# apcamargo/genomad

Hardware: NVIDIA H100
Metric: nn_classification_windows_per_s (higher is better)
Workload: dtype split operands on wgmma (conv: fp16 main pass + two e4m3 correction passes; w_v: 3 fp16 passes), fp32 accumulate; fp32-equivalent (<=1e-4 vs the fp32 oracle, measured ~1e-5)

## Files before the change

### genomad_b200/csrc/api.cu

```cuda
#include <cuda.h>
#include <cuda_runtime.h>
#include <cuda_fp16.h>

#include <algorithm>
#include <cmath>
#include <cstdio>
#include <cstring>
#include <string>
#include <vector>

#include "../../include/gnm.h"
#include "common.cuh"
#include "encode.cuh"
#include "conv_t.cuh"
#include "layer1_wv.cuh"
#include "conv_ref.cuh"
#include "igloo.cuh"
#include "dense.cuh"
#include "logits_tc.cuh"
#include "wv_gather.cuh"
#include "contigs.cuh"

using namespace gnm;

// ... 389 lines not shown
    if (dev_upload(h, &h->d1w, w->dense1_kernel, static_cast<size_t>(kHidden) * kHidden)) return 1;
    if (dev_upload(h, &h->d1b, w->dense1_bias, kHidden)) return 1;
    if (bn(w->bn1, &h->bn1_scale, &h->bn1_shift)) return 1;
    const float* dw[2] = {w->dense0_kernel, w->dense1_kernel};
    const int dk[2] = {256, kHidden};
    for (int L = 0; L < 2; ++L) {
      std::vector<float> thi(static_cast<size_t>(kHidden) * dk[L]), tlo(thi.size());
      for (int k = 0; k < dk[L]; ++k)
        for (int n = 0; n < kHidden; ++n)
          split_tf32(dw[L][static_cast<size_t>(k) * kHidden + n], thi[static_cast<size_t>(n) * dk[L] + k], tlo[static_cast<size_t>(n) * dk[L] + k]);
      if (dev_upload(h, &h->dwT_hi[L], thi.data(), thi.size())) return 1;
      if (dev_upload(h, &h->dwT_lo[L], tlo.data(), tlo.size())) return 1;
    }
    if (dev_upload(h, &h->d2w, w->dense2_kernel, static_cast<size_t>(kHidden) * 3)) return 1;
    if (dev_upload(h, &h->d2b, w->dense2_bias, 3)) return 1;
  }
  const size_t mb = static_cast<size_t>(max_batch);
  h->mb_pad = (max_batch + kBandWins - 1) / kBandWins * kBandWins;
  const size_t mbp = static_cast<size_t>(h->mb_pad);
  for (int i = 0; i < 2; ++i) {
    if (dev_alloc(h, &h->ybuf[i], mbp * kTok * kRowBytes)) return 1;
    for (int par = 0; par < 2; ++par) {
      if (dev_alloc(h, &h->q_set[par][i], mb * kPooled * kC)) return 1;
      if (dev_alloc(h, &h->mpi_set[par][i], mb * kPatches)) return 1;
      if (dev_alloc(h, &h->mpi_hi_set[par][i], mb * kPatches)) return 1;
      if (dev_alloc(h, &h->mpi_lo_set[par][i], mb * kPatches)) return 1;
    }
    h->q[i] = h->q_set[0][i]; h->mpi[i] = h->mpi_set[0][i]; h->mpi_hi[i] = h->mpi_hi_set[0][i]; h->mpi_lo[i] = h->mpi_lo_set[0][i];
    if (dev_alloc(h, &h->in_stage[i], mb * kWindow)) return 1;
    if (dev_alloc(h, &h->out_stage[i], mb * 3)) return 1;
    GNM_CUDA(cudaEventCreateWithFlags(&h->in_ready[i], cudaEventDisableTiming));
    GNM_CUDA(cudaEventCreateWithFlags(&h->in_free[i], cudaEventDisableTiming));
  }
  if (dev_alloc(h, &h->conv_dbg, static_cast<size_t>(h->num_sms) * 8)) return 1;
  GNM_CUDA(cudaMemset(h->conv_dbg, 0, static_cast<size_t>(h->num_sms) * 8 * sizeof(long long)));
  if (dev_alloc(h, &h->part, mbp * kGsSlots)) return 1;
  if (dev_alloc(h, &h->cta_split, static_cast<size_t>(2) * (h->num_sms + 1))) return 1;
  if (dev_alloc(h, &h->logits, mb * kLogitsLd)) return 1;
  if (dev_alloc(h, &h->logits_part, mb * kLogitsLd * kLgSplits)) return 1;
  if (dev_alloc(h, &h->h0, mb * 256)) return 1;
  if (dev_alloc(h, &h->h1, mb * kHidden)) return 1;
  if (dev_alloc(h, &h->h2, mb * kHidden)) return 1;
  if (dev_alloc(h, &h->hA_hi[0], mb * 256)) return 1;
  if (dev_alloc(h, &h->hA_lo[0], mb * 256)) return 1;
  if (dev_alloc(h, &h->hA_hi[1], mb * kHidden)) return 1;
  if (dev_alloc(h, &h->hA_lo[1], mb * kHidden)) return 1;
  GNM_CUDA(cudaStreamCreateWithFlags(&h->copy_stream, cudaStreamNonBlocking));
  GNM_CUDA(cudaStreamCreateWithFlags(&h->compute_stream, cudaStreamNonBlocking));
  {
    int prio_lo = 0, prio_hi = 0;
    GNM_CUDA(cudaDeviceGetStreamPriorityRange(&prio_lo, &prio_hi));
    GNM_CUDA(cudaStreamCreateWithPriority(&h->tail_stream, cudaStreamNonBlocking, prio_hi));
    for (int i = 0; i < 2; ++i) {
      GNM_CUDA(cudaEventCreateWithFlags(&h->main_done[i], cudaEventDisableTiming));
      GNM_CUDA(cudaEventCreateWithFlags(&h->tail_done[i], cudaEventDisableTiming));
    }
  }
  GNM_CUDA(cudaHostAlloc(reinterpret_cast<void**>(&h->status), sizeof(DeviceStatus), cudaHostAllocMapped));
  std::memset(h->status, 0, sizeof(DeviceStatus));

  PFN_encodeTiled enc = nullptr;
  if (get_encode_fn(&enc)) return 1;
  for (int i = 0; i < 2; ++i) {
    if (make_act_map(enc, &h->tm_act[i], h->ybuf[i], max_batch)) return 1;
    if (make_band_map(enc, &h->tm_band[i], h->ybuf[i], h->mb_pad)) return 1;
  }
  for (int i = 0; i < 4; ++i) {
    const int n_stages = i < 2 ? kConvStages : kWvStages;
// ... 90 lines not shown
    cfg.blockDim = dim3(kConvThreads); cfg.dynamicSmemBytes = kConvTSmem; cfg.stream = st; cfg.attrs = attr; cfg.numAttrs = 1;
    cfg.gridDim = dim3(grid / h->conv_cluster * h->conv_cluster);
    int max_clusters = 0;
    if (cudaOccupancyMaxActiveClusters(&max_clusters, conv_t_kernel<false>, &cfg) == cudaSuccess && max_clusters > 0)
      grid = std::min(grid / h->conv_cluster, max_clusters) * h->conv_cluster;
    else
      grid = grid / h->conv_cluster * h->conv_cluster;
    cfg.gridDim = dim3(grid);
    GNM_CUDA(cudaLaunchKernelEx(&cfg, conv_t_kernel<false>, h->tm_act[in_buf], h->tm_w_half[layer], p));
    return check_launch(h, "conv_t_kernel<false>(cluster)");
  }
  conv_t_kernel<false><<<grid, kConvThreads, kConvTSmem, st>>>(h->tm_act[in_buf], h->tm_w_half[layer], p);
  return check_launch(h, "conv_t_kernel<false>");
}
static int launch_wv_tc(gnm_handle* h, int s, int buf, int n, cudaStream_t st) {
  ConvTcParams p;
  p.status = h->status;
  p.experiment = 0;
  p.dbg = nullptr;
  p.bias = nullptr; p.y_out = nullptr; p.q_out = h->q[s];
  p.out_scale = h->wv_out_scale[s];
  p.out_fp8 = 0;
  p.n_tiles = n * kUnitsPerWin;
  const int grid = std::min(h->num_sms, p.n_tiles);
  conv_t_kernel<true><<<grid, kConvThreads, kConvTSmem, st>>>(h->tm_act[buf], h->tm_w_half[2 + s], p);
  return check_launch(h, "conv_t_kernel<true>");
}

static int wv_split(gnm_handle* h, int s, int groups, int grid, cudaStream_t st) {
  if (h->split_groups[s] == groups && h->split_grid[s] == grid) return 0;
  std::vector<double> cost(kNumBands);
  double total = 0;
  for (int b = 0; b < kNumBands; ++b) {
    const int per_warp = (h->band_groups[s][b] + kWgWarps - 1) / kWgWarps;
    cost[b] = h->wv_cost_base + h->wv_cost_group * per_warp;
    total += cost[b] * groups;
  }
  std::vector<int32_t>& sp = h->split_host[s];
  sp.assign(h->num_sms + 1, kNumBands * groups);
  sp[0] = 0;
  double acc = 0;
  int c = 1;
  for (int b = 0; b < kNumBands && c < grid; ++b)
    for (int g = 0; g < groups && c < grid; ++g) {
      acc += cost[b];
      if (acc >= total * c / grid) sp[c++] = b * groups + g + 1;
    }
  for (; c <= grid; ++c) sp[c] = kNumBands * groups;
  for (int i = 1; i <= grid; ++i) sp[i] = std::max(sp[i], sp[i - 1]);
  GNM_CUDA(cudaMemcpyAsync(h->cta_split + s * (h->num_sms + 1), sp.data(), (grid + 1) * sizeof(int32_t), cudaMemcpyHostToDevice, st));
  h->split_groups[s] = groups; h->split_grid[s] = grid;
  return 0;
}

static int launch_wv_gather(gnm_handle* h, int s, int buf, int n, cudaStream_t st) {
  WvGatherParams p;
  p.q_out = h->q[s]; p.out_scale = h->wv_out_scale[s];
  p.grp = h->grp[s]; p.band_gstart = h->band_gstart[s]; p.wfrag = h->wfrag[s]; p.gather_unscale = h->gather_unscale[s]; p.part_t = h->part;
  p.n_windows = n;
  p.n_pad = (n + kBandWins - 1) / kBandWins * kBandWins;
  p.groups = p.n_pad / kBandWins;
  p.n_units = kNumBands * p.groups;
  p.status = h->status;
  p.experiment = h->conv_experiment;
  p.dbg = (h->conv_experiment & 512) && s == 1 ? h->conv_dbg : nullptr;
  const int grid = std::min(h->num_sms, p.n_units);
  if (wv_split(h, s, p.groups, grid, st)) return 1;
// ... 535 lines not shown
  if (ns < 2) return 0;
  GNM_CUDA(cudaEventSynchronize(h->timer.events[ns - 1]));
  int k = 0;
  for (int i = 0; i + 1 < ns && k < cap; ++i) {
    if (std::strcmp(h->timer.names[i], "end") == 0) continue;
    float t = 0.f;
    GNM_CUDA(cudaEventElapsedTime(&t, h->timer.events[i], h->timer.events[i + 1]));
    if (names) names[k] = h->timer.names[i];
    if (ms) ms[k] = t;
    ++k;
  }
  *count = k;
  return 0;
}

extern "C" int gnm_debug_fetch(gnm_handle* h, const char* which, int n, float* d_dst, void* stream) {
  if (!h || !which || !d_dst) return fail("null argument");
  if (n < 1 || n > h->max_batch) return fail("gnm_debug_fetch: n out of range");
  GNM_CUDA(cudaSetDevice(h->device));
  cudaStream_t st = static_cast<cudaStream_t>(stream);
  const std::string k(which);
  const float* src = nullptr;
  size_t count = 0;
  if (k == "buf0" || k == "buf1") {
    const size_t rows = static_cast<size_t>(n) * kTok;
    join_rows_kernel<<<static_cast<unsigned>((rows * kC + 255) / 256), 256, 0, st>>>(h->ybuf[k == "buf1"], d_dst, rows,
                                                                                     h->ybuf_fp8lo[k == "buf1"]);
    return check_launch(h, "join_rows_kernel");
  } else if (k == "q0" || k == "q1") { src = h->q[k == "q1"]; count = static_cast<size_t>(n) * kPooled * kC; }
  else if (k == "mpi0" || k == "mpi1") { src = h->mpi[k == "mpi1"]; count = static_cast<size_t>(n) * kPatches; }
  else if (k == "h0") { src = h->h0; count = static_cast<size_t>(n) * 256; }
  else if (k == "h1" || k == "h2") { src = k == "h1" ? h->h1 : h->h2; count = static_cast<size_t>(n) * kHidden; }
  else if (k == "logits") { src = h->logits; count = static_cast<size_t>(n) * kLogitsLd; }
  else if (k == "conv_dbg") { src = reinterpret_cast<const float*>(h->conv_dbg); count = static_cast<size_t>(h->num_sms) * 16; }
  else return fail("gnm_debug_fetch: unknown buffer " + k);
  GNM_CUDA(cudaMemcpyAsync(d_dst, src, count * sizeof(float), cudaMemcpyDeviceToDevice, st));
  return 0;
}
```

### genomad_b200/csrc/common.cuh

```cuda
#pragma once
#include <cuda_runtime.h>
#include <cuda_fp16.h>
#include <cuda_fp8.h>
#include <stdint.h>
#include "wgmma.cuh"

namespace gnm {

constexpr int kWindow   = 6000;
constexpr int kTok      = 5997;
constexpr int kVocab    = 257;
constexpr int kC        = 128;
constexpr int kTaps     = 6;
constexpr int kPatches  = 2100;
constexpr int kPatchLen = 4;
constexpr int kPool     = 8;
constexpr int kPooled   = 749;
constexpr int kHidden   = 512;
constexpr float kLeaky  = 0.1f;

constexpr int kRowBytes  = 768;
constexpr int kOffHi16   = 0, kOffLo16 = 256, kOffP8 = 512;
constexpr float kActScale = 32.f;
constexpr float kLo8Scale = 128.f;
// ... 6 lines not shown
}
__device__ __forceinline__ float lrelu(float x) { return x > 0.f ? x : x * kLeaky; }

__device__ __forceinline__ void split_f16(float x, __half& hi, __half& lo) {
  hi = __float2half_rn(x);
  lo = __float2half_rn(x - __half2float(hi));
}
__device__ __forceinline__ uint32_t pack_h2(__half a, __half b) {
  return static_cast<uint32_t>(__half_as_ushort(a)) | (static_cast<uint32_t>(__half_as_ushort(b)) << 16);
}

__device__ __forceinline__ void split2_f16(float a, float b, __half2& hi, __half2& lo) {
  hi = __floats2half2_rn(a, b);
  const float2 f = __half22float2(hi);
  lo = __floats2half2_rn(a - f.x, b - f.y);
}

__device__ __forceinline__ uint16_t pack_e4m3x2(float a, float b) {
  return static_cast<uint16_t>(__nv_cvt_float2_to_fp8x2(make_float2(a, b), __NV_SATFINITE, __NV_E4M3));
}

__device__ __forceinline__ void stmatrix_x4_trans(uint32_t saddr, uint32_t r0, uint32_t r1, uint32_t r2, uint32_t r3) {
  asm volatile("stmatrix.sync.aligned.m8n8.x4.trans.shared.b16 [%0], {%1, %2, %3, %4};"
               ::"r"(saddr), "r"(r0), "r"(r1), "r"(r2), "r"(r3) : "memory");
}
__device__ __forceinline__ uint4 ld_shared_v4(uint32_t saddr) {
  uint4 v;
  asm volatile("ld.shared.v4.b32 {%0, %1, %2, %3}, [%4];" : "=r"(v.x), "=r"(v.y), "=r"(v.z), "=r"(v.w) : "r"(saddr) : "memory");
  return v;
}

struct DeviceStatus { int code; int info0; int info1; int info2; int act_overflow; int ov_stage[4]; };
enum : int { kDevOk = 0, kDevMbarTimeout = 1 };
__device__ __forceinline__ void flag_act_overflow(DeviceStatus* st, float absmax, float limit, int stage) {
  if (absmax > limit && st) { st->act_overflow = 1; st->ov_stage[stage] = 1; }
}

__device__ __forceinline__ bool elect_one() {
  uint32_t pred;
  asm volatile(
      "{\n\t.reg .pred P;\n\t"
      "elect.sync _|P, 0xffffffff;\n\t"
      "selp.u32 %0, 1, 0, P;\n\t}"
      : "=r"(pred));
  return pred != 0;
}

__device__ __forceinline__ void mbar_init(uint64_t* bar, uint32_t count) {
  asm volatile("mbarrier.init.shared::cta.b64 [%0], %1;" ::"r"(smem_u32(bar)), "r"(count));
}
__device__ __forceinline__ void fence_barrier_init() {
  asm volatile("fence.mbarrier_init.release.cluster;" ::: "memory");
}
__device__ __forceinline__ void fence_proxy_async_smem() {
  asm volatile("fence.proxy.async.shared::cta;" ::: "memory");
}
__device__ __forceinline__ void mbar_arrive_expect_tx(uint64_t* bar, uint32_t bytes) {
  asm volatile("mbarrier.arrive.expect_tx.shared::cta.b64 _, [%0], %1;" ::"r"(smem_u32(bar)), "r"(bytes) : "memory");
}
__device__ __forceinline__ void mbar_arrive(uint64_t* bar) {
  asm volatile("mbarrier.arrive.shared::cta.b64 _, [%0];" ::"r"(smem_u32(bar)) : "memory");
}
__device__ __forceinline__ bool mbar_try_wait(uint64_t* bar, uint32_t parity) {
  uint32_t ok;
  asm volatile(
      "{\n\t.reg .pred p;\n\t"
// ... 45 lines not shown
```

### genomad_b200/csrc/conv_t.cuh

```cuda
#pragma once
#include <cuda.h>
#include "common.cuh"

namespace gnm {

constexpr int kTileM       = 128;
constexpr int kUnitsPerWin = (kTok + 2 * kTileM - 1) / (2 * kTileM);
constexpr int kSlabRows    = 136;
constexpr int kARegion     = kSlabRows * 128;
constexpr int kA2Region    = 2 * kARegion;
constexpr int kNumRegions  = 4;
constexpr int kA2Bytes     = kNumRegions * kA2Region;
constexpr int kBStage      = 128 * 128;
constexpr int kBHalf       = kBStage / 2;
constexpr int kConvThreads = 384;
constexpr int kConvStages  = 24;
constexpr int kWvStages    = 4;
constexpr int kTWSlots     = 5;
constexpr int kEpiTile     = 512;
constexpr int kEpiStage    = 8 * 2 * kEpiTile;
constexpr int kConvTSmem   = kA2Bytes + 2 * kTWSlots * kBHalf + kEpiStage + 2048;
static_assert(kConvTSmem <= 232448, "conv_t_kernel exceeds the 227 KB of shared memory a CTA may use");

struct ConvTcParams {
// ... 180 lines not shown
        for (int j = 0; j < 32; ++j) {
          uint32_t r[4];
#pragma unroll
          for (int h = 0; h < 2; ++h) {
            const float bias = h ? bias1 : bias0;
            const float y0 = kActScale * lrelu(fmaf(d[4 * j + 2 * h], oscale, bias));
            const float y1 = kActScale * lrelu(fmaf(d[4 * j + 2 * h + 1], oscale, bias));
            amax = fmaxf(amax, fmaxf(fabsf(y0), fabsf(y1)));
            if (p.out_fp8) {
              const __half2 hh = __floats2half2_rn(y0, y1);
              const float2 f = __half22float2(hh);
              const uint32_t e0 = pack_e4m3x2((y0 - f.x) * kLo8Scale, f.x * kHi8Scale);
              const uint32_t e1 = pack_e4m3x2((y1 - f.y) * kLo8Scale, f.y * kHi8Scale);
              r[h] = pack_h2(__low2half(hh), __high2half(hh));
              r[2 + h] = e0 | (e1 << 16);
            } else {
              __half2 hh, l;
              split2_f16(y0, y1, hh, l);
              r[h] = pack_h2(__low2half(hh), __high2half(hh));
              r[2 + h] = pack_h2(__low2half(l), __high2half(l));
            }
          }
          const uint32_t buf = (j & 1) * kEpiTile;
          stmatrix_x4_trans(st_addr + buf, r[0], r[1], r[2], r[3]);
          __syncwarp();
          const uint4 v = ld_shared_v4(ld_addr + buf);
          if (store && t0 + 8 * j + lp < kTok) *reinterpret_cast<uint4*>(dst + static_cast<size_t>(8 * j) * kRowBytes) = v;
        }
      }
      t_epi += clock64() - tq;
    }
    if (!kWvMode) flag_act_overflow(p.status, amax, p.out_fp8 ? kHi8Limit : kF16Limit, p.out_fp8 ? 2 : 3);
    if (p.dbg && wq == 0 && lane == 0) {
      long long* dd = p.dbg + blockIdx.x * 8;
      if (g == 0) { dd[0] = clock64() - t_begin; dd[1] = t_mma; dd[2] = w_a; dd[3] = w_w; dd[4] = it; dd[6] = t_epi; }
      else { dd[5] = t_mma; dd[7] = t_epi; }
    }
  }
}

}
```

### genomad_b200/csrc/wv_gather.cuh

```cuda
#pragma once
#include <cuda.h>
#include <type_traits>
#include "common.cuh"
#include "conv_t.cuh"
#include "igloo.cuh"

namespace gnm {

constexpr int kBandRows   = 24;
constexpr int kBandWins   = 8;
constexpr int kWgN        = kBandRows * kBandWins;
constexpr int kNumBands   = (kTok + kBandRows - 1) / kBandRows;
constexpr int kWgRegion   = kWgN * 128;
constexpr int kWgBufs     = 6;
constexpr int kWgSlab     = kWgBufs * kWgRegion;
constexpr int kWgWBytes   = kWvStages * kBStage;
constexpr int kWgMmaWarps = 8;
constexpr int kWgWarps    = 7;
constexpr int kWgThreads  = (kWgMmaWarps + kWgWarps + 1) * 32;
constexpr int kWgGroupCap = 4;
constexpr int kWgGroupMax = 4;
constexpr int kWgSmem     = kWgSlab + kWgWBytes + 2048;
static_assert(kWgSmem <= 232448, "wv_gather_kernel exceeds the 227 KB of shared memory a CTA may use");
static_assert(kWgN == 3 * 64 && kBandRows == 3 * kPool && kBandWins == 8, "unit shape: three pool groups of 8 positions x 8 windows");
static_assert(kWgRegion % 1024 == 0, "regions must keep the 1024-byte alignment of the 128-byte swizzle");

struct WvGatherParams {
  float* q_out;
  float out_scale;
  const int2* grp;
  const int32_t* band_gstart;
  const uint4* wfrag;
  float gather_unscale;
  float* part_t;
  int n_windows, n_pad;
  int groups;
  int n_units;
  const int32_t* cta_split;
  int experiment;
  long long* dbg;
  DeviceStatus* status;
};

__device__ __forceinline__ uint2 ldg_frag(const uint2* p) {
  uint2 v;
  asm volatile("ld.global.nc.L1::evict_last.v2.u32 {%0, %1}, [%2];" : "=r"(v.x), "=r"(v.y) : "l"(p));
  return v;
}
__device__ __forceinline__ void ldsm_x4(uint32_t saddr, uint32_t (&a)[4]) {
  asm volatile("ldmatrix.sync.aligned.m8n8.x4.shared.b16 {%0, %1, %2, %3}, [%4];"
               : "=r"(a[0]), "=r"(a[1]), "=r"(a[2]), "=r"(a[3]) : "r"(saddr));
}
__device__ __forceinline__ void mma_16816(float (&d)[4], const uint32_t (&a)[4], uint32_t b0, uint32_t b1) {
  asm volatile("mma.sync.aligned.m16n8k16.row.col.f32.f16.f16.f32 {%0, %1, %2, %3}, {%4, %5, %6, %7}, {%8, %9}, {%0, %1, %2, %3};"
               : "+f"(d[0]), "+f"(d[1]), "+f"(d[2]), "+f"(d[3]) : "r"(a[0]), "r"(a[1]), "r"(a[2]), "r"(a[3]), "r"(b0), "r"(b1));
}

__global__ void __launch_bounds__(kWgThreads, 1)
wv_gather_kernel(const __grid_constant__ CUtensorMap tm_band, const __grid_constant__ CUtensorMap tm_w, const WvGatherParams p) {
  extern __shared__ uint8_t smem_raw[];
  uint8_t* smem = reinterpret_cast<uint8_t*>((reinterpret_cast<uintptr_t>(smem_raw) + 1023) & ~uintptr_t(1023));
  uint8_t* s_a = smem;
  uint8_t* s_w = smem + kWgSlab;
  uint64_t* bars = reinterpret_cast<uint64_t*>(s_w + kWgWBytes);
  uint64_t* a_full = bars;
  uint64_t* a_empty = bars + 8;
  uint64_t* w_full = bars + 16;

  const int warp = __shfl_sync(0xffffffffu, static_cast<int>(threadIdx.x) >> 5, 0);
  const int lane = threadIdx.x & 31;
  constexpr int kProducerWarp = kWgMmaWarps + kWgWarps;
  const int u_begin = p.cta_split[blockIdx.x], u_end = p.cta_split[blockIdx.x + 1];

  if (warp == kProducerWarp && elect_one()) {
    tma_prefetch_desc(&tm_band);
    tma_prefetch_desc(&tm_w);
    for (int i = 0; i < kWgBufs; ++i) { mbar_init(&a_full[i], 1); mbar_init(&a_empty[i], kWgMmaWarps + kWgWarps); }
    mbar_init(w_full, 1);
    fence_barrier_init();
  }
  __syncthreads();

  if (warp == kProducerWarp) {
    if (elect_one()) {
      mbar_arrive_expect_tx(w_full, kWgWBytes);
      for (int q = 0; q < kWvStages; ++q) tma_load_2d_hint(s_w + q * kBStage, &tm_w, w_full, 0, q * 128, l2_policy_evict_last());
      const uint64_t pol = l2_policy_evict_first();
      uint32_t phases = 0;
      int b0 = 0;
      long long c_wait_empty = 0;
      for (int unit = u_begin; unit < u_end; ++unit) {
        const int band = unit / p.groups;
        const int w0 = (unit - band * p.groups) * kBandWins;
#pragma unroll
        for (int k = 0; k < 4; ++k) {
          int b = b0 + k; if (b >= kWgBufs) b -= kWgBufs;
          const long long tq = clock64();
          mbar_wait(&a_empty[b], ((phases >> b) & 1) ^ 1, p.status, 500 + b);
          c_wait_empty += clock64() - tq;
          phases ^= 1u << b;
          mbar_arrive_expect_tx(&a_full[b], kWgRegion);
          const int src = (k & 1 ? kOffLo16 : kOffHi16) + (k >> 1) * 128;
          tma_load_3d_hint(s_a + b * kWgRegion, &tm_band, &a_full[b], src, w0, band * kBandRows, pol);
        }
        b0 += 4; if (b0 >= kWgBufs) b0 -= kWgBufs;
      }
      if (p.dbg) p.dbg[blockIdx.x * 8 + 7] = c_wait_empty;
    }
  } else if (warp < kWgMmaWarps) {
    const int g = warp >> 2, wq = warp & 3;
    const uint32_t a_base = smem_u32(s_a);
    const uint32_t w_base = smem_u32(s_w) + g * 64 * 128;
    const int ch0 = g * 64 + wq * 16 + (lane >> 2);
    const int win0 = 2 * (lane & 3);
    const float oscale = p.out_scale;
    mbar_wait(w_full, 0, p.status, 510);
    uint32_t phases = 0;
    int b0 = 0;
    uint32_t w_a = 0, t_mma = 0, t_epi = 0;
    float d[96];
    for (int unit = u_begin; unit < u_end; ++unit) {
      auto buf = [&](int k) { const int b = b0 + k; return b >= kWgBufs ? b - kWgBufs : b; };
      const uint32_t t_unit = clock();
#pragma unroll
      for (int kh = 0; kh < 2; ++kh) {
#pragma unroll
        for (int r = 0; r < 2; ++r) {
          const int b = buf(2 * kh + r);
          const uint32_t tq = clock();
          mbar_wait(&a_full[b], (phases >> b) & 1, p.status, 530 + b);
          w_a += clock() - tq;
          phases ^= 1u << b;
        }
        const uint64_t yh = gmma_desc_sw128(a_base + buf(2 * kh) * kWgRegion);
        const uint64_t yl = gmma_desc_sw128(a_base + buf(2 * kh + 1) * kWgRegion);
        const uint64_t whi = gmma_desc_sw128(w_base + (2 * kh) * kBStage);
        const uint64_t wlo = gmma_desc_sw128(w_base + (2 * kh + 1) * kBStage);
        wgmma_fence();
#pragma unroll
        for (int kk = 0; kk < 4; ++kk) {
          wgmma_f16_n192(d, whi + kk * 2, yh + kk * 2, (kh == 0 && kk == 0) ? 0u : 1u);
          wgmma_f16_n192(d, whi + kk * 2, yl + kk * 2, 1u);
        }
#pragma unroll
        for (int kk = 0; kk < 4; ++kk) wgmma_f16_n192(d, wlo + kk * 2, yh + kk * 2, 1u);
        wgmma_commit();
      }
      wgmma_wait<1>();
      __syncwarp();
      if (lane == 0) { mbar_arrive(&a_empty[buf(0)]); mbar_arrive(&a_empty[buf(1)]); }
      wgmma_wait<0>();
      wgmma_fence_regs(d);
      const uint32_t t_epi0 = clock();
      t_mma += t_epi0 - t_unit;
      const int band = unit / p.groups;
      const int w0 = (unit - band * p.groups) * kBandWins;
#pragma unroll
      for (int pg = 0; pg < kBandRows / kPool; ++pg) {
        const int gg = band * (kBandRows / kPool) + pg;
        if (gg < kPooled && !(p.experiment & 128)) {
#pragma unroll
          for (int h = 0; h < 2; ++h)
#pragma unroll
            for (int e = 0; e < 2; ++e) {
              float m = d[32 * pg + 2 * h + e];
#pragma unroll
              for (int i = 1; i < kPool; ++i) m = fmaxf(m, d[32 * pg + 4 * i + 2 * h + e]);
              const int w = w0 + win0 + e;
              if (w < p.n_windows) p.q_out[(static_cast<size_t>(w) * kPooled + gg) * kC + ch0 + 8 * h] = m * oscale;
            }
        }
      }
      __syncwarp();
      if (lane == 0) { mbar_arrive(&a_empty[buf(2)]); mbar_arrive(&a_empty[buf(3)]); }
      t_epi += clock() - t_epi0;
      b0 += 4; if (b0 >= kWgBufs) b0 -= kWgBufs;
    }
    if (p.dbg && warp == 0 && lane == 0) { long long* o = p.dbg + blockIdx.x * 8; o[3] = t_mma; o[4] = w_a; o[6] = t_epi; }
  } else {
    const int gw = warp - kWgMmaWarps;
    const float gscale = p.gather_unscale;
    const int lm_plane = (lane >> 3) & 1, lm_chunk = lane >> 4, lm_win = lane & 7;
    const int gid = lane >> 2, tig = lane & 3;
    const uint32_t slab = smem_u32(s_a);
    int it = 0;
    uint32_t phases = 0;
    int b0 = 0;
    long long c_wait_full = 0, c_gather = 0, tq = 0;
    const long long t_begin = clock64();
    int cur_band = -1, g_first = 0, g_cnt = 0, n_mine = 0;
    int my_e0[kWgGroupCap] = {}, my_meta[kWgGroupCap] = {};
    bool fast = true;
    struct GroupFrag { uint2 b[4]; uint32_t a[4][4]; };
    auto load_group = [&](int e0, int meta, int kh, uint32_t hi_base, uint32_t lo_base, GroupFrag& f) {
      const int row = meta & 31, ne = meta >> 8;
      const uint2* wf = reinterpret_cast<const uint2*>(p.wfrag) + ((static_cast<size_t>(e0 + (gid >> 1)) * 2 + kh) * 16 + tig) * 2 + (gid & 1);
#pragma unroll
      for (int ks = 0; ks < 4; ++ks) f.b[ks] = ((gid >> 1) < ne && !(p.experiment & 1024)) ? ldg_frag(wf + ks * 8) : make_uint2(0u, 0u);
      const uint32_t rb = (lm_plane ? lo_base : hi_base) + row * (kBandWins * 128) + lm_win * 128;
#pragma unroll
      for (int ks = 0; ks < 4; ++ks) {
        if (p.experiment & 2048) { f.a[ks][0] = f.a[ks][1] = f.a[ks][2] = f.a[ks][3] = rb; continue; }
        ldsm_x4(rb + (((ks * 2 + lm_chunk) ^ lm_win) << 4), f.a[ks]);
      }
    };
    auto mma_group = [&](const GroupFrag& f) -> float {
      float d[4][4];
#pragma unroll
      for (int ks = 0; ks < 4; ++ks) d[ks][0] = d[ks][1] = d[ks][2] = d[ks][3] = 0.f;
      if (p.experiment & 256) {
#pragma unroll
        for (int ks = 0; ks < 4; ++ks) asm volatile("" :: "r"(f.a[ks][0] | f.a[ks][1] | f.a[ks][2] | f.a[ks][3] | f.b[ks].x | f.b[ks].y));
      } else {
#pragma unroll
        for (int ks = 0; ks < 4; ++ks) mma_16816(d[ks], f.a[ks], f.b[ks].x, f.b[ks].y);
      }
      float v = 0.f;
#pragma unroll
      for (int ks = 0; ks < 4; ++ks) v += (d[ks][0] + d[ks][2]) + (d[ks][1] + d[ks][3]);
      return v * gscale;
    };
    for (int unit = u_begin; unit < u_end; ++unit, ++it) {
      const int band = unit / p.groups;
      const int w0 = (unit - band * p.groups) * kBandWins;
      if (band != cur_band) {
        cur_band = band;
        g_first = p.band_gstart[band];
        g_cnt = (p.experiment & 32) ? 0 : p.band_gstart[band + 1] - g_first;
        fast = g_cnt <= kWgWarps * kWgGroupCap;
        n_mine = 0;
#pragma unroll
        for (int i = 0; i < kWgGroupCap; ++i) {
          const int gi = gw + i * kWgWarps;
          if (fast && gi < g_cnt) { const int2 m = p.grp[g_first + gi]; my_e0[i] = m.x; my_meta[i] = m.y; n_mine = i + 1; }
        }
      }
      float c0[kWgGroupCap];
#pragma unroll 1
      for (int kh = 0; kh < 2; ++kh) {
        int bh = b0 + 2 * kh; if (bh >= kWgBufs) bh -= kWgBufs;
        int bl = b0 + 2 * kh + 1; if (bl >= kWgBufs) bl -= kWgBufs;
        const uint32_t ph_h = (phases >> bh) & 1, ph_l = (phases >> bl) & 1;
        phases ^= (1u << bh) | (1u << bl);
        const uint32_t hi_base = slab + bh * kWgRegion, lo_base = slab + bl * kWgRegion;
        if (p.dbg) tq = clock64();
        mbar_wait(&a_full[bh], ph_h, p.status, 550 + bh);
        mbar_wait(&a_full[bl], ph_l, p.status, 560 + bl);
        if (p.dbg) { const long long t = clock64(); c_wait_full += t - tq; tq = t; }
        if (fast) {
          auto finish = [&](int i, float v) {
            if (kh == 0) c0[i] = v;
            else if (tig < (my_meta[i] >> 8) && !(p.experiment & 64))
              p.part_t[static_cast<size_t>(my_e0[i] + tig) * p.n_pad + w0 + gid] = c0[i] + v;
          };
#pragma unroll
          for (int i = 0; i < kWgGroupCap; i += 2)
            if (i < n_mine) {
              GroupFrag f0, f1;
              load_group(my_e0[i], my_meta[i], kh, hi_base, lo_base, f0);
              if (i + 1 < n_mine) {
                load_group(my_e0[i + 1], my_meta[i + 1], kh, hi_base, lo_base, f1);
                finish(i, mma_group(f0));
                finish(i + 1, mma_group(f1));
              } else {
                finish(i, mma_group(f0));
              }
            }
        } else {
#pragma unroll 1
          for (int gi = gw; gi < g_cnt; gi += kWgWarps) {
            const int2 m = p.grp[g_first + gi];
            GroupFrag f;
            load_group(m.x, m.y, kh, hi_base, lo_base, f);
            const float v = mma_group(f);
            if (tig < (m.y >> 8)) {
              float* gp = p.part_t + static_cast<size_t>(m.x + tig) * p.n_pad + w0 + gid;
              *gp = kh == 0 ? v : *gp + v;
            }
          }
        }
        __syncwarp();
        if (lane == 0) { mbar_arrive(&a_empty[bh]); mbar_arrive(&a_empty[bl]); }
        if (p.dbg) c_gather += clock64() - tq;
      }
      b0 += 4; if (b0 >= kWgBufs) b0 -= kWgBufs;
    }
    if (p.dbg && warp == kWgMmaWarps && lane == 0) {
      long long* d = p.dbg + blockIdx.x * 8;
      d[0] = clock64() - t_begin; d[1] = c_wait_full; d[2] = c_gather; d[5] = it;
    }
  }
}

__global__ void __launch_bounds__(256)
patch_finish_t_kernel(const float* __restrict__ part_t, const int32_t* __restrict__ slot_of, const float* __restrict__ w_bias,
                      float* __restrict__ mpi, float* __restrict__ mpi_hi, float* __restrict__ mpi_lo, int n_windows, int n_pad) {
  __shared__ float tile[32][33];
  const int p0 = blockIdx.x * 32, w0 = blockIdx.y * 32;
  const int tx = threadIdx.x & 31, ty = threadIdx.x >> 5;
  for (int pp = ty; pp < 32; pp += 8) {
    const int pch = p0 + pp, w = w0 + tx;
    float v = 0.f;
    if (pch < kPatches && w < n_windows) {
      const int4 s4 = *reinterpret_cast<const int4*>(slot_of + pch * 4);
      v = (((part_t[static_cast<size_t>(s4.x) * n_pad + w] + part_t[static_cast<size_t>(s4.y) * n_pad + w]) +
            part_t[static_cast<size_t>(s4.z) * n_pad + w]) + part_t[static_cast<size_t>(s4.w) * n_pad + w]) + w_bias[pch];
    }
    tile[pp][tx] = v;
  }
  __syncthreads();
  for (int ww = ty; ww < 32; ww += 8) {
    const int pch = p0 + tx, w = w0 + ww;
    if (pch < kPatches && w < n_windows) {
      const float v = tile[tx][ww];
      const size_t o = static_cast<size_t>(w) * kPatches + pch;
      mpi[o] = v;
      const float hi = __uint_as_float(__float_as_uint(v) & 0xffffe000u);
      mpi_hi[o] = hi;
      mpi_lo[o] = __uint_as_float(__float_as_uint(v - hi) & 0xffffe000u);
    }
  }
}
// ... 3 lines not shown
```

### genomad_b200/engine.py

```python
from __future__ import annotations

import ctypes as C
import os
from pathlib import Path
from typing import Dict, List, NamedTuple, Optional, Tuple

import numpy as np

from . import weights as _weights

_PKG = Path(__file__).resolve().parent
_LIB_PATH = Path(os.environ["GENOMAD_B200_LIB"]) if os.environ.get("GENOMAD_B200_LIB") else _PKG / "libgnm.so"
_lib = None

WINDOW = 6000
TOKENS = 5997
EMBED = 512


class GnmError(RuntimeError):
    pass


class _IglooW(C.Structure):
# ... 349 lines not shown
        contig = t.repeat_interleave(t.arange(n, dtype=t.int32, device=seq.device), counts)
        probs = (self.predict_windows(seq, start, length) if start.numel()
                 else t.zeros((0, 3), dtype=t.float32, device=seq.device))
        rel = start - offs[:-1].index_select(0, contig.to(t.int64)) if start.numel() else start
        return WindowScores(probs, contig, rel, length, woff)

    def classify_host(self, ascii_windows: np.ndarray) -> np.ndarray:
        a = np.ascontiguousarray(ascii_windows, dtype=np.uint8)
        assert a.ndim == 2 and a.shape[1] == WINDOW
        out = np.empty((a.shape[0], 3), dtype=np.float32)
        with self._torch.cuda.device(self.device):
            _check(self.lib, self.lib.gnm_classify_host(self._h, _ptr(a), a.shape[0], _ptr(out)))
        return out

    def classify_host_into(self, ascii_ptr: int, n: int, out_ptr: int):
        with self._torch.cuda.device(self.device):
            _check(self.lib, self.lib.gnm_classify_host(self._h, ascii_ptr, n, out_ptr))

    def check_status(self):
        _check(self.lib, self.lib.gnm_check_status(self._h, self._stream()))

    def stage_times(self) -> List[Tuple[str, float]]:
        cap = 16384
        names = (C.c_char_p * cap)()
        ms = (C.c_float * cap)()
        cnt = C.c_int(cap)
        _check(self.lib, self.lib.gnm_stage_times(self._h, names, ms, C.byref(cnt)))
        return [(names[i].decode(), float(ms[i])) for i in range(cnt.value)]

    def debug_fetch(self, which: str, n: int):
        t = self._torch
        shapes = {"buf0": (n, TOKENS, 128), "buf1": (n, TOKENS, 128), "q0": (n, 749, 128), "q1": (n, 749, 128),
                  "mpi0": (n, 2100), "mpi1": (n, 2100), "h0": (n, 256), "h1": (n, 512), "h2": (n, 512), "logits": (n, 752),
                  "conv_dbg": (self.get_option("num_sms"), 16)}
        out = t.empty(shapes[which], dtype=t.float32, device=self._dev())
        _check(self.lib, self.lib.gnm_debug_fetch(self._h, which.encode(), n, out.data_ptr(), self._stream()))
        return out
```

Baseline: 56960.

## Share w_v patch gather across MMA warps and rebalance registers with setmaxnreg

The patch-gather work, previously done only by 7 dedicated gather warps, is now split across those warps plus the 8 wgmma consumer warps. The consumer warps run their share between wgmma commit and wait, overlapping tensor-core latency with mma.sync gather work. setmaxnreg raises registers for the MMA warps and lowers them for producer/gather warps, and the per-warp group cap drops from 4 to 2. The change adds register pressure in the MMA warps, releases the first A-buffers later, and needs a matching cost-model update in the host split plus a larger debug-slot array.

```diff
diff --git a/genomad_b200/csrc/api.cu b/genomad_b200/csrc/api.cu
--- a/genomad_b200/csrc/api.cu
+++ b/genomad_b200/csrc/api.cu
@@ -445,8 +445,8 @@
     GNM_CUDA(cudaEventCreateWithFlags(&h->in_ready[i], cudaEventDisableTiming));
     GNM_CUDA(cudaEventCreateWithFlags(&h->in_free[i], cudaEventDisableTiming));
   }
-  if (dev_alloc(h, &h->conv_dbg, static_cast<size_t>(h->num_sms) * 8)) return 1;
-  GNM_CUDA(cudaMemset(h->conv_dbg, 0, static_cast<size_t>(h->num_sms) * 8 * sizeof(long long)));
+  if (dev_alloc(h, &h->conv_dbg, static_cast<size_t>(h->num_sms) * kDbgSlots)) return 1;
+  GNM_CUDA(cudaMemset(h->conv_dbg, 0, static_cast<size_t>(h->num_sms) * kDbgSlots * sizeof(long long)));
   if (dev_alloc(h, &h->part, mbp * kGsSlots)) return 1;
   if (dev_alloc(h, &h->cta_split, static_cast<size_t>(2) * (h->num_sms + 1))) return 1;
   if (dev_alloc(h, &h->logits, mb * kLogitsLd)) return 1;
@@ -603,7 +603,7 @@
   std::vector<double> cost(kNumBands);
   double total = 0;
   for (int b = 0; b < kNumBands; ++b) {
-    const int per_warp = (h->band_groups[s][b] + kWgWarps - 1) / kWgWarps;
+    const int per_warp = (h->band_groups[s][b] + kWgGatherWarps - 1) / kWgGatherWarps;
     cost[b] = h->wv_cost_base + h->wv_cost_group * per_warp;
     total += cost[b] * groups;
   }
@@ -1205,7 +1205,7 @@
   else if (k == "h0") { src = h->h0; count = static_cast<size_t>(n) * 256; }
   else if (k == "h1" || k == "h2") { src = k == "h1" ? h->h1 : h->h2; count = static_cast<size_t>(n) * kHidden; }
   else if (k == "logits") { src = h->logits; count = static_cast<size_t>(n) * kLogitsLd; }
-  else if (k == "conv_dbg") { src = reinterpret_cast<const float*>(h->conv_dbg); count = static_cast<size_t>(h->num_sms) * 16; }
+  else if (k == "conv_dbg") { src = reinterpret_cast<const float*>(h->conv_dbg); count = static_cast<size_t>(h->num_sms) * kDbgSlots * 2; }
   else return fail("gnm_debug_fetch: unknown buffer " + k);
   GNM_CUDA(cudaMemcpyAsync(d_dst, src, count * sizeof(float), cudaMemcpyDeviceToDevice, st));
   return 0;
diff --git a/genomad_b200/csrc/common.cuh b/genomad_b200/csrc/common.cuh
--- a/genomad_b200/csrc/common.cuh
+++ b/genomad_b200/csrc/common.cuh
@@ -62,6 +62,7 @@
 
 struct DeviceStatus { int code; int info0; int info1; int info2; int act_overflow; int ov_stage[4]; };
 enum : int { kDevOk = 0, kDevMbarTimeout = 1 };
+constexpr int kDbgSlots = 16;
 __device__ __forceinline__ void flag_act_overflow(DeviceStatus* st, float absmax, float limit, int stage) {
   if (absmax > limit && st) { st->act_overflow = 1; st->ov_stage[stage] = 1; }
 }
diff --git a/genomad_b200/csrc/conv_t.cuh b/genomad_b200/csrc/conv_t.cuh
--- a/genomad_b200/csrc/conv_t.cuh
+++ b/genomad_b200/csrc/conv_t.cuh
@@ -236,7 +236,7 @@
     }
     if (!kWvMode) flag_act_overflow(p.status, amax, p.out_fp8 ? kHi8Limit : kF16Limit, p.out_fp8 ? 2 : 3);
     if (p.dbg && wq == 0 && lane == 0) {
-      long long* dd = p.dbg + blockIdx.x * 8;
+      long long* dd = p.dbg + blockIdx.x * kDbgSlots;
       if (g == 0) { dd[0] = clock64() - t_begin; dd[1] = t_mma; dd[2] = w_a; dd[3] = w_w; dd[4] = it; dd[6] = t_epi; }
       else { dd[5] = t_mma; dd[7] = t_epi; }
     }
diff --git a/genomad_b200/csrc/wv_gather.cuh b/genomad_b200/csrc/wv_gather.cuh
--- a/genomad_b200/csrc/wv_gather.cuh
+++ b/genomad_b200/csrc/wv_gather.cuh
@@ -18,7 +18,11 @@
 constexpr int kWgMmaWarps = 8;
 constexpr int kWgWarps    = 7;
 constexpr int kWgThreads  = (kWgMmaWarps + kWgWarps + 1) * 32;
-constexpr int kWgGroupCap = 4;
+constexpr int kWgGatherWarps = kWgWarps + kWgMmaWarps;
+constexpr int kWgGroupCap = 2;
+constexpr int kWgMmaRegs    = 152;
+constexpr int kWgGatherRegs = 104;
+static_assert(2 * 128 * (kWgMmaRegs + kWgGatherRegs) <= 65536 && kWgMmaRegs % 8 == 0 && kWgGatherRegs % 8 == 0, "setmaxnreg split");
 constexpr int kWgGroupMax = 4;
 constexpr int kWgSmem     = kWgSlab + kWgWBytes + 2048;
 static_assert(kWgSmem <= 232448, "wv_gather_kernel exceeds the 227 KB of shared memory a CTA may use");
@@ -55,6 +59,8 @@
   asm volatile("mma.sync.aligned.m16n8k16.row.col.f32.f16.f16.f32 {%0, %1, %2, %3}, {%4, %5, %6, %7}, {%8, %9}, {%0, %1, %2, %3};"
                : "+f"(d[0]), "+f"(d[1]), "+f"(d[2]), "+f"(d[3]) : "r"(a[0]), "r"(a[1]), "r"(a[2]), "r"(a[3]), "r"(b0), "r"(b1));
 }
+template <int kRegs> __device__ __forceinline__ void setmaxnreg_inc() { asm volatile("setmaxnreg.inc.sync.aligned.u32 %0;" ::"n"(kRegs)); }
+template <int kRegs> __device__ __forceinline__ void setmaxnreg_dec() { asm volatile("setmaxnreg.dec.sync.aligned.u32 %0;" ::"n"(kRegs)); }
 
 __global__ void __launch_bounds__(kWgThreads, 1)
 wv_gather_kernel(const __grid_constant__ CUtensorMap tm_band, const __grid_constant__ CUtensorMap tm_w, const WvGatherParams p) {
@@ -81,33 +87,96 @@
   }
   __syncthreads();
 
-  if (warp == kProducerWarp) {
-    if (elect_one()) {
-      mbar_arrive_expect_tx(w_full, kWgWBytes);
-      for (int q = 0; q < kWvStages; ++q) tma_load_2d_hint(s_w + q * kBStage, &tm_w, w_full, 0, q * 128, l2_policy_evict_last());
-      const uint64_t pol = l2_policy_evict_first();
-      uint32_t phases = 0;
-      int b0 = 0;
-      long long c_wait_empty = 0;
-      for (int unit = u_begin; unit < u_end; ++unit) {
-        const int band = unit / p.groups;
-        const int w0 = (unit - band * p.groups) * kBandWins;
-#pragma unroll
-        for (int k = 0; k < 4; ++k) {
-          int b = b0 + k; if (b >= kWgBufs) b -= kWgBufs;
-          const long long tq = clock64();
-          mbar_wait(&a_empty[b], ((phases >> b) & 1) ^ 1, p.status, 500 + b);
-          c_wait_empty += clock64() - tq;
-          phases ^= 1u << b;
-          mbar_arrive_expect_tx(&a_full[b], kWgRegion);
-          const int src = (k & 1 ? kOffLo16 : kOffHi16) + (k >> 1) * 128;
-          tma_load_3d_hint(s_a + b * kWgRegion, &tm_band, &a_full[b], src, w0, band * kBandRows, pol);
-        }
-        b0 += 4; if (b0 >= kWgBufs) b0 -= kWgBufs;
-      }
-      if (p.dbg) p.dbg[blockIdx.x * 8 + 7] = c_wait_empty;
-    }
-  } else if (warp < kWgMmaWarps) {
+  const int gslot = warp < kWgMmaWarps ? kWgWarps + warp : warp - kWgMmaWarps;
+  const int lm_plane = (lane >> 3) & 1, lm_chunk = lane >> 4, lm_win = lane & 7;
+  const int gid = lane >> 2, tig = lane & 3;
+  const float gscale = p.gather_unscale;
+  int cur_band = -1, g_first = 0, g_cnt = 0, n_mine = 0;
+  int my_e0[kWgGroupCap] = {}, my_meta[kWgGroupCap] = {};
+  bool fast = true;
+  float c0[kWgGroupCap];
+  auto take_band = [&](int band) {
+    if (band == cur_band) return;
+    cur_band = band;
+    g_first = p.band_gstart[band];
+    g_cnt = (p.experiment & 32) ? 0 : p.band_gstart[band + 1] - g_first;
+    fast = g_cnt <= kWgGatherWarps * kWgGroupCap;
+    n_mine = 0;
+#pragma unroll
+    for (int i = 0; i < kWgGroupCap; ++i) {
+      const int gi = gslot + i * kWgGatherWarps;
+      if (fast && gi < g_cnt) { const int2 m = p.grp[g_first + gi]; my_e0[i] = m.x; my_meta[i] = m.y; n_mine = i + 1; }
+    }
+  };
+  struct GroupFrag { uint2 b[4]; uint32_t a[4][4]; };
+  auto load_group = [&](int e0, int meta, int kh, uint32_t hi_base, uint32_t lo_base, GroupFrag& f) {
+    const int row = meta & 31, ne = meta >> 8;
+    const uint2* wf = reinterpret_cast<const uint2*>(p.wfrag) + ((static_cast<size_t>(e0 + (gid >> 1)) * 2 + kh) * 16 + tig) * 2 + (gid & 1);
+#pragma unroll
+    for (int ks = 0; ks < 4; ++ks) f.b[ks] = ((gid >> 1) < ne && !(p.experiment & 1024)) ? ldg_frag(wf + ks * 8) : make_uint2(0u, 0u);
+    const uint32_t rb = (lm_plane ? lo_base : hi_base) + row * (kBandWins * 128) + lm_win * 128;
+#pragma unroll
+    for (int ks = 0; ks < 4; ++ks) {
+      if (p.experiment & 2048) { f.a[ks][0] = f.a[ks][1] = f.a[ks][2] = f.a[ks][3] = rb; continue; }
+      ldsm_x4(rb + (((ks * 2 + lm_chunk) ^ lm_win) << 4), f.a[ks]);
+    }
+  };
+  auto mma_group = [&](const GroupFrag& f) -> float {
+    float d[4][4];
+#pragma unroll
+    for (int ks = 0; ks < 4; ++ks) d[ks][0] = d[ks][1] = d[ks][2] = d[ks][3] = 0.f;
+    if (p.experiment & 256) {
+#pragma unroll
+      for (int ks = 0; ks < 4; ++ks) asm volatile("" :: "r"(f.a[ks][0] | f.a[ks][1] | f.a[ks][2] | f.a[ks][3] | f.b[ks].x | f.b[ks].y));
+    } else {
+#pragma unroll
+      for (int ks = 0; ks < 4; ++ks) mma_16816(d[ks], f.a[ks], f.b[ks].x, f.b[ks].y);
+    }
+    float v = 0.f;
+#pragma unroll
+    for (int ks = 0; ks < 4; ++ks) v += (d[ks][0] + d[ks][2]) + (d[ks][1] + d[ks][3]);
+    return v * gscale;
+  };
+  auto gather = [&](int kh, uint32_t hi_base, uint32_t lo_base, int w0, bool paired) {
+    if (fast) {
+      auto finish = [&](int i, float v) {
+        if (kh == 0) c0[i] = v;
+        else if (tig < (my_meta[i] >> 8) && !(p.experiment & 64))
+          p.part_t[static_cast<size_t>(my_e0[i] + tig) * p.n_pad + w0 + gid] = c0[i] + v;
+      };
+      static_assert(kWgGroupCap == 2, "the fast path handles at most two groups per warp");
+      if (n_mine > 0) {
+        GroupFrag f0, f1;
+        load_group(my_e0[0], my_meta[0], kh, hi_base, lo_base, f0);
+        if (n_mine > 1 && paired) {
+          load_group(my_e0[1], my_meta[1], kh, hi_base, lo_base, f1);
+          finish(0, mma_group(f0));
+          finish(1, mma_group(f1));
+        } else {
+          finish(0, mma_group(f0));
+          if (n_mine > 1) {
+            load_group(my_e0[1], my_meta[1], kh, hi_base, lo_base, f1);
+            finish(1, mma_group(f1));
+          }
+        }
+      }
+    } else {
+#pragma unroll 1
+      for (int gi = gslot; gi < g_cnt; gi += kWgGatherWarps) {
+        const int2 m = p.grp[g_first + gi];
+        GroupFrag f;
+        load_group(m.x, m.y, kh, hi_base, lo_base, f);
+        const float v = mma_group(f);
+        if (tig < (m.y >> 8)) {
+          float* gp = p.part_t + static_cast<size_t>(m.x + tig) * p.n_pad + w0 + gid;
+          *gp = kh == 0 ? v : *gp + v;
+        }
+      }
+    }
+  };
+
+  if (warp < kWgMmaWarps) {
+    setmaxnreg_inc<kWgMmaRegs>();
     const int g = warp >> 2, wq = warp & 3;
     const uint32_t a_base = smem_u32(s_a);
     const uint32_t w_base = smem_u32(s_w) + g * 64 * 128;
@@ -117,10 +186,13 @@
     mbar_wait(w_full, 0, p.status, 510);
     uint32_t phases = 0;
     int b0 = 0;
-    uint32_t w_a = 0, t_mma = 0, t_epi = 0;
+    uint32_t w_a = 0, t_mma = 0, t_epi = 0, t_gat = 0, w_mma = 0;
     float d[96];
     for (int unit = u_begin; unit < u_end; ++unit) {
       auto buf = [&](int k) { const int b = b0 + k; return b >= kWgBufs ? b - kWgBufs : b; };
+      const int band = unit / p.groups;
+      const int w0 = (unit - band * p.groups) * kBandWins;
+      take_band(band);
       const uint32_t t_unit = clock();
 #pragma unroll
       for (int kh = 0; kh < 2; ++kh) {
@@ -146,15 +218,25 @@
         for (int kk = 0; kk < 4; ++kk) wgmma_f16_n192(d, wlo + kk * 2, yh + kk * 2, 1u);
         wgmma_commit();
       }
+      uint32_t tg = clock();
+      gather(0, a_base + buf(0) * kWgRegion, a_base + buf(1) * kWgRegion, w0, false);
+      uint32_t tw = clock();
+      t_gat += tw - tg;
       wgmma_wait<1>();
+      tg = clock();
+      w_mma += tg - tw;
       __syncwarp();
       if (lane == 0) { mbar_arrive(&a_empty[buf(0)]); mbar_arrive(&a_empty[buf(1)]); }
+      gather(1, a_base + buf(2) * kWgRegion, a_base + buf(3) * kWgRegion, w0, false);
+      tw = clock();
+      t_gat += tw - tg;
       wgmma_wait<0>();
       wgmma_fence_regs(d);
       const uint32_t t_epi0 = clock();
+      w_mma += t_epi0 - tw;
       t_mma += t_epi0 - t_unit;
-      const int band = unit / p.groups;
-      const int w0 = (unit - band * p.groups) * kBandWins;
+      __syncwarp();
+      if (lane == 0) { mbar_arrive(&a_empty[buf(2)]); mbar_arrive(&a_empty[buf(3)]); }
 #pragma unroll
       for (int pg = 0; pg < kBandRows / kPool; ++pg) {
         const int gg = band * (kBandRows / kPool) + pg;
@@ -171,123 +253,73 @@
             }
         }
       }
-      __syncwarp();
-      if (lane == 0) { mbar_arrive(&a_empty[buf(2)]); mbar_arrive(&a_empty[buf(3)]); }
       t_epi += clock() - t_epi0;
       b0 += 4; if (b0 >= kWgBufs) b0 -= kWgBufs;
     }
-    if (p.dbg && warp == 0 && lane == 0) { long long* o = p.dbg + blockIdx.x * 8; o[3] = t_mma; o[4] = w_a; o[6] = t_epi; }
+    if (p.dbg && warp == 0 && lane == 0) {
+      long long* o = p.dbg + blockIdx.x * kDbgSlots;
+      o[3] = t_mma; o[4] = w_a; o[6] = t_epi; o[8] = t_gat; o[9] = w_mma;
+    }
   } else {
-    const int gw = warp - kWgMmaWarps;
-    const float gscale = p.gather_unscale;
-    const int lm_plane = (lane >> 3) & 1, lm_chunk = lane >> 4, lm_win = lane & 7;
-    const int gid = lane >> 2, tig = lane & 3;
-    const uint32_t slab = smem_u32(s_a);
-    int it = 0;
-    uint32_t phases = 0;
-    int b0 = 0;
-    long long c_wait_full = 0, c_gather = 0, tq = 0;
-    const long long t_begin = clock64();
-    int cur_band = -1, g_first = 0, g_cnt = 0, n_mine = 0;
-    int my_e0[kWgGroupCap] = {}, my_meta[kWgGroupCap] = {};
-    bool fast = true;
-    struct GroupFrag { uint2 b[4]; uint32_t a[4][4]; };
-    auto load_group = [&](int e0, int meta, int kh, uint32_t hi_base, uint32_t lo_base, GroupFrag& f) {
-      const int row = meta & 31, ne = meta >> 8;
-      const uint2* wf = reinterpret_cast<const uint2*>(p.wfrag) + ((static_cast<size_t>(e0 + (gid >> 1)) * 2 + kh) * 16 + tig) * 2 + (gid & 1);
-#pragma unroll
-      for (int ks = 0; ks < 4; ++ks) f.b[ks] = ((gid >> 1) < ne && !(p.experiment & 1024)) ? ldg_frag(wf + ks * 8) : make_uint2(0u, 0u);
-      const uint32_t rb = (lm_plane ? lo_base : hi_base) + row * (kBandWins * 128) + lm_win * 128;
-#pragma unroll
-      for (int ks = 0; ks < 4; ++ks) {
-        if (p.experiment & 2048) { f.a[ks][0] = f.a[ks][1] = f.a[ks][2] = f.a[ks][3] = rb; continue; }
-        ldsm_x4(rb + (((ks * 2 + lm_chunk) ^ lm_win) << 4), f.a[ks]);
-      }
-    };
-    auto mma_group = [&](const GroupFrag& f) -> float {
-      float d[4][4];
-#pragma unroll
-      for (int ks = 0; ks < 4; ++ks) d[ks][0] = d[ks][1] = d[ks][2] = d[ks][3] = 0.f;
-      if (p.experiment & 256) {
-#pragma unroll
-        for (int ks = 0; ks < 4; ++ks) asm volatile("" :: "r"(f.a[ks][0] | f.a[ks][1] | f.a[ks][2] | f.a[ks][3] | f.b[ks].x | f.b[ks].y));
-      } else {
-#pragma unroll
-        for (int ks = 0; ks < 4; ++ks) mma_16816(d[ks], f.a[ks], f.b[ks].x, f.b[ks].y);
-      }
-      float v = 0.f;
-#pragma unroll
-      for (int ks = 0; ks < 4; ++ks) v += (d[ks][0] + d[ks][2]) + (d[ks][1] + d[ks][3]);
-      return v * gscale;
-    };
-    for (int unit = u_begin; unit < u_end; ++unit, ++it) {
-      const int band = unit / p.groups;
-      const int w0 = (unit - band * p.groups) * kBandWins;
-      if (band != cur_band) {
-        cur_band = band;
-        g_first = p.band_gstart[band];
-        g_cnt = (p.experiment & 32) ? 0 : p.band_gstart[band + 1] - g_first;
-        fast = g_cnt <= kWgWarps * kWgGroupCap;
-        n_mine = 0;
-#pragma unroll
-        for (int i = 0; i < kWgGroupCap; ++i) {
-          const int gi = gw + i * kWgWarps;
-          if (fast && gi < g_cnt) { const int2 m = p.grp[g_first + gi]; my_e0[i] = m.x; my_meta[i] = m.y; n_mine = i + 1; }
-        }
-      }
-      float c0[kWgGroupCap];
+    setmaxnreg_dec<kWgGatherRegs>();
+    if (warp == kProducerWarp) {
+      if (elect_one()) {
+        mbar_arrive_expect_tx(w_full, kWgWBytes);
+        for (int q = 0; q < kWvStages; ++q) tma_load_2d_hint(s_w + q * kBStage, &tm_w, w_full, 0, q * 128, l2_policy_evict_last());
+        const uint64_t pol = l2_policy_evict_first();
+        uint32_t phases = 0;
+        int b0 = 0;
+        long long c_wait_empty = 0;
+        for (int unit = u_begin; unit < u_end; ++unit) {
+          const int band = unit / p.groups;
+          const int w0 = (unit - band * p.groups) * kBandWins;
+#pragma unroll
+          for (int k = 0; k < 4; ++k) {
+            int b = b0 + k; if (b >= kWgBufs) b -= kWgBufs;
+            const long long tq = clock64();
+            mbar_wait(&a_empty[b], ((phases >> b) & 1) ^ 1, p.status, 500 + b);
+            c_wait_empty += clock64() - tq;
+            phases ^= 1u << b;
+            mbar_arrive_expect_tx(&a_full[b], kWgRegion);
+            const int src = (k & 1 ? kOffLo16 : kOffHi16) + (k >> 1) * 128;
+            tma_load_3d_hint(s_a + b * kWgRegion, &tm_band, &a_full[b], src, w0, band * kBandRows, pol);
+          }
+          b0 += 4; if (b0 >= kWgBufs) b0 -= kWgBufs;
+        }
+        if (p.dbg) p.dbg[blockIdx.x * kDbgSlots + 7] = c_wait_empty;
+      }
+    } else {
+      const uint32_t slab = smem_u32(s_a);
+      int it = 0;
+      uint32_t phases = 0;
+      int b0 = 0;
+      long long c_wait_full = 0, c_gather = 0, tq = 0;
+      const long long t_begin = clock64();
+      for (int unit = u_begin; unit < u_end; ++unit, ++it) {
+        const int band = unit / p.groups;
+        const int w0 = (unit - band * p.groups) * kBandWins;
+        take_band(band);
 #pragma unroll 1
-      for (int kh = 0; kh < 2; ++kh) {
-        int bh = b0 + 2 * kh; if (bh >= kWgBufs) bh -= kWgBufs;
-        int bl = b0 + 2 * kh + 1; if (bl >= kWgBufs) bl -= kWgBufs;
-        const uint32_t ph_h = (phases >> bh) & 1, ph_l = (phases >> bl) & 1;
-        phases ^= (1u << bh) | (1u << bl);
-        const uint32_t hi_base = slab + bh * kWgRegion, lo_base = slab + bl * kWgRegion;
-        if (p.dbg) tq = clock64();
-        mbar_wait(&a_full[bh], ph_h, p.status, 550 + bh);
-        mbar_wait(&a_full[bl], ph_l, p.status, 560 + bl);
-        if (p.dbg) { const long long t = clock64(); c_wait_full += t - tq; tq = t; }
-        if (fast) {
-          auto finish = [&](int i, float v) {
-            if (kh == 0) c0[i] = v;
-            else if (tig < (my_meta[i] >> 8) && !(p.experiment & 64))
-              p.part_t[static_cast<size_t>(my_e0[i] + tig) * p.n_pad + w0 + gid] = c0[i] + v;
-          };
-#pragma unroll
-          for (int i = 0; i < kWgGroupCap; i += 2)
-            if (i < n_mine) {
-              GroupFrag f0, f1;
-              load_group(my_e0[i], my_meta[i], kh, hi_base, lo_base, f0);
-              if (i + 1 < n_mine) {
-                load_group(my_e0[i + 1], my_meta[i + 1], kh, hi_base, lo_base, f1);
-                finish(i, mma_group(f0));
-                finish(i + 1, mma_group(f1));
-              } else {
-                finish(i, mma_group(f0));
-              }
-            }
-        } else {
-#pragma unroll 1
-          for (int gi = gw; gi < g_cnt; gi += kWgWarps) {
-            const int2 m = p.grp[g_first + gi];
-            GroupFrag f;
-            load_group(m.x, m.y, kh, hi_base, lo_base, f);
-            const float v = mma_group(f);
-            if (tig < (m.y >> 8)) {
-              float* gp = p.part_t + static_cast<size_t>(m.x + tig) * p.n_pad + w0 + gid;
-              *gp = kh == 0 ? v : *gp + v;
-            }
-          }
-        }
-        __syncwarp();
-        if (lane == 0) { mbar_arrive(&a_empty[bh]); mbar_arrive(&a_empty[bl]); }
-        if (p.dbg) c_gather += clock64() - tq;
-      }
-      b0 += 4; if (b0 >= kWgBufs) b0 -= kWgBufs;
-    }
-    if (p.dbg && warp == kWgMmaWarps && lane == 0) {
-      long long* d = p.dbg + blockIdx.x * 8;
-      d[0] = clock64() - t_begin; d[1] = c_wait_full; d[2] = c_gather; d[5] = it;
+        for (int kh = 0; kh < 2; ++kh) {
+          int bh = b0 + 2 * kh; if (bh >= kWgBufs) bh -= kWgBufs;
+          int bl = b0 + 2 * kh + 1; if (bl >= kWgBufs) bl -= kWgBufs;
+          const uint32_t ph_h = (phases >> bh) & 1, ph_l = (phases >> bl) & 1;
+          phases ^= (1u << bh) | (1u << bl);
+          if (p.dbg) tq = clock64();
+          mbar_wait(&a_full[bh], ph_h, p.status, 550 + bh);
+          mbar_wait(&a_full[bl], ph_l, p.status, 560 + bl);
+          if (p.dbg) { const long long t = clock64(); c_wait_full += t - tq; tq = t; }
+          gather(kh, slab + bh * kWgRegion, slab + bl * kWgRegion, w0, true);
+          __syncwarp();
+          if (lane == 0) { mbar_arrive(&a_empty[bh]); mbar_arrive(&a_empty[bl]); }
+          if (p.dbg) c_gather += clock64() - tq;
+        }
+        b0 += 4; if (b0 >= kWgBufs) b0 -= kWgBufs;
+      }
+      if (p.dbg && warp == kWgMmaWarps && lane == 0) {
+        long long* d = p.dbg + blockIdx.x * kDbgSlots;
+        d[0] = clock64() - t_begin; d[1] = c_wait_full; d[2] = c_gather; d[5] = it;
+      }
     }
   }
 }
diff --git a/genomad_b200/engine.py b/genomad_b200/engine.py
--- a/genomad_b200/engine.py
+++ b/genomad_b200/engine.py
@@ -405,7 +405,7 @@
         t = self._torch
         shapes = {"buf0": (n, TOKENS, 128), "buf1": (n, TOKENS, 128), "q0": (n, 749, 128), "q1": (n, 749, 128),
                   "mpi0": (n, 2100), "mpi1": (n, 2100), "h0": (n, 256), "h1": (n, 512), "h2": (n, 512), "logits": (n, 752),
-                  "conv_dbg": (self.get_option("num_sms"), 16)}
+                  "conv_dbg": (self.get_option("num_sms"), 32)}
         out = t.empty(shapes[which], dtype=t.float32, device=self._dev())
         _check(self.lib, self.lib.gnm_debug_fetch(self._h, which.encode(), n, out.data_ptr(), self._stream()))
         return out
```

New measurement: 58290, median of 6. 2.3% higher.
